# ydixon/yolo_v3

Hardware: AMD Instinct MI355X
Metric: images/sec (YOLOv3 forward + decode + NMS, 416x416, bs=64 per GPU) (higher is better)
Workload: dtype f32 (exact fp32 MFMA); 1 GPU; 416x416 bs=64 per GPU, 64 distinct synthetic scenes per GPU, SW-1 synthetic weights, conf=0.50 nms=0.40; global_batch=64, parallelism=dp1, entry=Detector.run_device, lanes=2

## Files before the change

### include/yv3.h

```cpp
#ifndef YV3_H
#define YV3_H

#include <stddef.h>
#include <stdint.h>

#ifdef __cplusplus
extern "C" {
#endif

#define YV3_VERSION 100

#define YV3_EINVAL   (-1)
#define YV3_ESHAPE   (-2)
#define YV3_EWORKSPACE (-3)
#define YV3_EDTYPE   (-4)
#define YV3_ERCCL    (-5)
#define YV3_ELIMIT   (-6)

#define YV3_F32  0
#define YV3_BF16 1
#define YV3_F32_BF16X3 2
#define YV3_F32_F16X2 3

#define YV3_ACT_LINEAR 0
#define YV3_ACT_LEAKY  1

int yv3_version(void);
const char* yv3_error_string(int code);


int yv3_pack_conv_weight(const float* w_oihw, void* w_packed, int cout, int cin, int k,
                         int cout_pad, int dtype, void* stream);

int yv3_fold_bn(const float* gamma, const float* bias, const float* mean, const float* var,
                float eps, float* alpha, float* beta, int channels, void* stream);

int yv3_split_planes(const float* in, void* out, long long n, int np, void* stream);
int yv3_merge_planes(const void* in, float* out, long long n, int np, void* stream);


int yv3_conv0(const float* x_nchw, const float* w_tap_major, const float* alpha, const float* beta,
              void* y_nhwc, int B, int H, int W, int out_dtype, int* flags, void* stream);

int yv3_conv_front(const float* x_nchw, const float* w0_tap_major, const float* alpha0, const float* beta0,
                   const void* w1_packed, const float* alpha1, const float* beta1, void* y,
                   int B, int H, int W, int* flags, void* stream);
int yv3_conv_front_bf16(const float* x_nchw, const float* w0_tap_major, const float* alpha0, const float* beta0,
                        const void* w1_packed, const float* alpha1, const float* beta1, void* y,
                        int B, int H, int W, int* flags, void* stream);
int yv3_conv_front_f32(const float* x_nchw, const float* w0_tap_major, const float* alpha0, const float* beta0,
                       const float* w1_packed, const float* alpha1, const float* beta1, float* y,
                       int B, int H, int W, void* stream);

int yv3_res_block64(const void* x, const void* w1_packed, const float* alpha1, const float* beta1,
                    const void* w2_packed, const float* alpha2, const float* beta2, void* y,
                    int B, int H, int W, int* flags, void* stream);
int yv3_res_block64_bf16(const void* x, const void* w1_packed, const float* alpha1, const float* beta1,
                         const void* w2_packed, const float* alpha2, const float* beta2, void* y,
                         int B, int H, int W, int* flags, void* stream);
int yv3_res_block64_f32(const float* x, const float* w1_packed, const float* alpha1, const float* beta1,
                        const float* w2_packed, const float* alpha2, const float* beta2, float* y,
                        int B, int H, int W, void* stream);

typedef struct yv3_conv_desc {
    const void*  x;
    const void*  x2;
    const void*  w;
    const float* alpha;
    const float* beta;
    const void*  residual;
    void*        y;
    int B, H, W;
    int cin;
    int cin_up;
    int cout, cout_pad;
    int k, stride;
    int act;
    int dtype;
    int out_dtype;
    int* flags;
    void*  workspace;
    size_t workspace_bytes;
    float*    dec_out;
    long long dec_out_batch_stride;
    float     dec_stride;
    float     dec_anchors[6];
    unsigned  options;
    int       big_tile_min;
    int       tune[4];
    long long x_plane_stride, x2_plane_stride, y_plane_stride;
    const void*  w_wino;
    const float* alpha_wino;
    void*        wino_ws;
    size_t       wino_ws_bytes;
    const void*  w_wino4;
} yv3_conv_desc;

#define YV3_OPT_NO_PINGPONG 1u
#define YV3_OPT_K3S1        2u
#define YV3_OPT_WINO_EVEN   4u
#define YV3_OPT_WINO_ALWAYS 8u
#define YV3_OPT_TWO_LANES   16u
#define YV3_OPT_WINO4_TILES 32u
#define YV3_OPT_TILE_SHIFT  8

size_t yv3_conv_workspace_bytes(void);

size_t yv3_wino_workspace_bytes(int B, int H, int W, int cin);

size_t yv3_wino4_workspace_bytes(int B, int H, int W, int cin);
int yv3_pack_wino4_weight_f32(const float* u_oc66, float* packed, int cout, int cin, void* stream);

int yv3_conv2d(const yv3_conv_desc* desc, void* stream);

#define YV3_FORM_DIRECT   0
#define YV3_FORM_WINOGRAD 1
#define YV3_FORM_WINOGRAD4 2
int yv3_conv2d_form(const yv3_conv_desc* desc);

int yv3_conv2d_launches(const yv3_conv_desc* desc);

int yv3_conv2d_kernel(const yv3_conv_desc* desc, char* buf, size_t buf_bytes);

int yv3_conv2d_sequence(const yv3_conv_desc* descs, int n, void* stream);


int yv3_decode(const float* logits, int ld_logits, const float* anchors_host, float stride,
               float* out, long long out_batch_stride, int B, int H, int W, int num_class,
               void* stream);

int yv3_decode_nchw(const float* logits_nchw, const float* anchors_host, float stride,
                    float* out, long long out_batch_stride, int B, int H, int W, int num_class,
                    void* stream);


int yv3_cxcywh_to_xyxy(const float* in, float* out, long long n, void* stream);

int yv3_iou_matrix(const float* b1, int n1, int ld1, const float* b2, int n2, int ld2,
                   int mode, float* out, void* stream);


size_t yv3_postproc_cand_bytes(int B, int max_cand, int num_class);

size_t yv3_postproc_nms_workspace_bytes(int B, int max_n, int num_class);

#define YV3_PP_EVAL 1
#define YV3_PP_PROB 2

int yv3_postproc_filter(const float* dets, int B, int N, int num_class, float conf_thr,
                        int mode, void* cand, int max_cand, int* cand_counts, void* stream);

int yv3_postproc_nms(const float* dets, int B, int N, int num_class, float nms_thr, int use_nms,
                     const void* cand, int max_cand, const int* cand_counts, int max_n,
                     float* out_boxes, int cap, int* out_counts,
                     void* workspace, size_t workspace_bytes, void* stream);


int yv3_letterbox(const unsigned char* img_hwc, int H, int W, float* out_chw, int out_h, int out_w,
                  void* stream);

int yv3_letterbox_ex(const unsigned char* img_hwc, int H, int W, float* out_chw, int out_h, int out_w,
                     int box_w, int box_h, int box_x, int box_y, void* stream);

int yv3_resize_linear(const unsigned char* img_hwc, int H, int W, float* out_chw, int out_h, int out_w,
                      void* stream);

int yv3_correct_boxes(const float* boxes, int B, int cap, int ld, const int* counts, const int* org_wh,
                      int img_w, int img_h, int is_letterbox, int out_xyxy, float* out, void* stream);


size_t yv3_augment_workspace_bytes(long long src_bytes);

int yv3_augment_images(const unsigned char* src, long long src_bytes, const long long* offsets, const int* hw,
                       const double* params, int B, float* out, int out_h, int out_w,
                       void* workspace, size_t workspace_bytes, int* status, void* stream);

int yv3_augment_labels(const double* labels, int B, int T, const int* hw, const double* params,
                       float* target, int max_rows, int out_h, int out_w, int* status, void* stream);

int yv3_upsample2x_concat(const float* up, const float* tail, float* out, int B, int c_up, int c_tail, int h, int w, void* stream);

int yv3_gather_boxes(const float* payload, float* gathered, int b_local, int rows, void* rccl_comm, void* stream);

#define YV3_COCO_MAX_MAXDETS 8

typedef struct yv3_cocoeval_desc {
    int n_gt, n_det, n_img, n_cat;
    const int* gt_img;
    const int* gt_cat;
    const double* gt_box;
    const double* gt_area;
    const int* gt_crowd;
    const long long* gt_id;
    const int* det_img;
    const int* det_cat;
    const double* det_box;
    const double* det_score;
    int n_iou, n_rec, n_area, n_maxdet;
    const double* iou_thrs;
    const double* rec_thrs;
    const double* area_rng;
    int max_dets[YV3_COCO_MAX_MAXDETS];
    double* precision;
    double* recall;
    double* scores;
    int* status;
} yv3_cocoeval_desc;

size_t yv3_cocoeval_workspace_bytes(int n_gt, int n_det, int n_img, int n_cat, int n_area);

int yv3_cocoeval(const yv3_cocoeval_desc* desc, void* ws, size_t ws_bytes, void* stream);

#define YV3_YOLO_LOSS_MAX_ROWS 1024

typedef struct yv3_yolo_loss_desc {
    const float* logits;
    float* grad;
    long long stride_b, stride_p, stride_c;
    const float* target;
    int B, H, W, T, num_class;
    float img_dim_h;
    float anchors[18];
    int mask[3];
    double* sums;
    int* counts;
    int* status;
} yv3_yolo_loss_desc;

size_t yv3_yolo_loss_workspace_bytes(int B, int H, int W, int T);

int yv3_yolo_loss(const yv3_yolo_loss_desc* desc, void* ws, size_t ws_bytes, void* stream);


int yv3_train_pack_weight(const float* w, float* wf, float* wd, int cout, int cin, int k, void* stream);

int yv3_train_conv_fwd(const float* x, const float* x2, const float* wf, const float* bias, float* z,
                       int B, int H, int W, int cin, int cin_up, int cout, int k, int stride, int x_nchw, void* stream);

int yv3_train_conv_dgrad(const float* dz, const float* wd, float* dx, int B, int H, int W, int cin, int cout, int k, int stride,
                         int accumulate, void* stream);

size_t yv3_train_conv_wgrad_workspace_bytes(int B, int H, int W, int cin, int cout, int k, int stride);
int yv3_train_conv_wgrad(const float* x, const float* x2, const float* dz, float* dw, int B, int H, int W, int cin, int cin_up,
                         int cout, int k, int stride, int x_nchw, void* ws, size_t ws_bytes, void* stream);

size_t yv3_train_channel_workspace_bytes(long long P, int C);

int yv3_train_bn_stats(const float* z, long long P, int C, float eps, float momentum, const float* run_mean, const float* run_var,
                       float* run_mean_out, float* run_var_out, float* mean, float* invstd, void* ws, size_t ws_bytes, void* stream);

int yv3_train_bn_eval_stats(const float* run_mean, const float* run_var, float eps, float* mean, float* invstd, int C, void* stream);

int yv3_train_bn_act_fwd(const float* z, const float* mean, const float* invstd, const float* gamma, const float* beta,
                         const float* residual, float* y, long long P, int C, void* stream);

int yv3_train_bn_act_bwd(const float* z, const float* dy, const float* mean, const float* invstd, const float* gamma, const float* beta,
// ... 30 lines not shown
```

### yolo_v3_amd/_ffi.py

```python
import ctypes
import os

_HERE = os.path.dirname(os.path.abspath(__file__))
LIB_PATH = (os.environ.get("YV3_LIB") if os.environ.get("YV3_MEASURE") == "1" else None) or os.path.join(_HERE, "libyv3.so")

if os.environ.get("YV3_MEASURE") != "1":
    _stray = sorted(k for k in os.environ if k.startswith("YV3_") and k not in ("YV3_MEASURE", "YV3_DIST_BACKEND", "YV3_DUMP_PLAN"))
    if _stray:
        import warnings
        warnings.warn("yolo_v3_amd: %s set but ignored -- library / kernel-selection overrides are honoured in measurement sessions only "
                      "(YV3_MEASURE=1); the bundled libyv3.so and the default plans are used" % ", ".join(_stray), RuntimeWarning)

F32, BF16, F32X3, F32H2 = 0, 1, 2, 3
ACT_LINEAR, ACT_LEAKY = 0, 1
PP_EVAL, PP_PROB = 1, 2
OPT_NO_PINGPONG, OPT_K3S1, OPT_WINO_EVEN, OPT_WINO_ALWAYS, OPT_TWO_LANES, OPT_WINO4_TILES = 1, 2, 4, 8, 16, 32
OPT_TILE_SHIFT = 8
(TILE_AUTO, TILE_256x128_W8, TILE_128x128_W8, TILE_128x128_W4, TILE_128x64, TILE_256x128_W4, TILE_256x256, TILE_256x128_W4_ROLL,
 TILE_256x256_ROLL, TILE_256x256_ROLL4) = range(10)
TILE_192x256_ROLL, TILE_W4_192x128, TILE_256x256_PP3, TILE_256x256_PP4, TILE_192x256_PP3, TILE_192x256_PP4 = 11, 12, 13, 14, 15, 16
T0_F32_TILE_64, T0_F32_TILE_128_W4, T0_F32_TILE_128_1X1, T0_WINO2_HALF, T0_WINO2_FULL = 2, 6, 7, 8, 9
T0_WINO4_NEVER, T0_WINO4_ALWAYS, T0_GEMM_NEVER, T0_GEMM_ALWAYS = 10, 11, 13, 14
T1_WINO4_NO_EVEN, T1_WINO4_NO_FULL, T1_GEMM_ALL_ROWS = 1, 2, 3
T1P_NO_SHORT_K, T1P_WINO_OTHER_LOOP, T1P_BF16_ROUND3, T1P_BF16_NO_192, T1P_NO_W4 = 1, 2, 8, 16, 32
T1P_NO_W4_1X1, T1P_NO_W4_3X3, T1P_W4_LANES_3X3, T1P_BF16_ROLL, T1P_BF16_PP3 = 64, 128, 256, 512, 1024
KERNEL_LINE_BYTES = 96


def conv2d_kernel(desc):
    buf = ctypes.create_string_buffer(KERNEL_LINE_BYTES)
    check(lib().yv3_conv2d_kernel(ctypes.byref(desc), buf, KERNEL_LINE_BYTES), "yv3_conv2d_kernel")
    return buf.value.decode()

c_void_p, c_int, c_float, c_size_t, c_longlong = (ctypes.c_void_p, ctypes.c_int, ctypes.c_float,
                                                  ctypes.c_size_t, ctypes.c_longlong)


class ConvDesc(ctypes.Structure):
    _fields_ = [("x", c_void_p), ("x2", c_void_p), ("w", c_void_p), ("alpha", c_void_p), ("beta", c_void_p),
                ("residual", c_void_p), ("y", c_void_p),
                ("B", c_int), ("H", c_int), ("W", c_int), ("cin", c_int), ("cin_up", c_int),
                ("cout", c_int), ("cout_pad", c_int), ("k", c_int), ("stride", c_int), ("act", c_int),
                ("dtype", c_int), ("out_dtype", c_int), ("flags", c_void_p),
                ("workspace", c_void_p), ("workspace_bytes", ctypes.c_size_t),
                ("dec_out", c_void_p), ("dec_out_batch_stride", c_longlong), ("dec_stride", c_float),
                ("dec_anchors", c_float * 6), ("options", ctypes.c_uint), ("big_tile_min", c_int), ("tune", c_int * 4),
                ("x_plane_stride", c_longlong), ("x2_plane_stride", c_longlong), ("y_plane_stride", c_longlong),
                ("w_wino", c_void_p), ("alpha_wino", c_void_p), ("wino_ws", c_void_p), ("wino_ws_bytes", ctypes.c_size_t),
                ("w_wino4", c_void_p)]


COCO_MAX_MAXDETS = 8
ELIMIT = -6


class CocoEvalDesc(ctypes.Structure):
    _fields_ = [("n_gt", c_int), ("n_det", c_int), ("n_img", c_int), ("n_cat", c_int),
                ("gt_img", c_void_p), ("gt_cat", c_void_p), ("gt_box", c_void_p), ("gt_area", c_void_p),
                ("gt_crowd", c_void_p), ("gt_id", c_void_p),
                ("det_img", c_void_p), ("det_cat", c_void_p), ("det_box", c_void_p), ("det_score", c_void_p),
                ("n_iou", c_int), ("n_rec", c_int), ("n_area", c_int), ("n_maxdet", c_int),
                ("iou_thrs", c_void_p), ("rec_thrs", c_void_p), ("area_rng", c_void_p),
                ("max_dets", c_int * COCO_MAX_MAXDETS),
                ("precision", c_void_p), ("recall", c_void_p), ("scores", c_void_p), ("status", c_void_p)]


YOLO_LOSS_MAX_ROWS = 1024
EINVAL, ESHAPE, EWORKSPACE = -1, -2, -3


class YoloLossDesc(ctypes.Structure):
    _fields_ = [("logits", c_void_p), ("grad", c_void_p),
                ("stride_b", c_longlong), ("stride_p", c_longlong), ("stride_c", c_longlong),
                ("target", c_void_p), ("B", c_int), ("H", c_int), ("W", c_int), ("T", c_int), ("num_class", c_int),
                ("img_dim_h", c_float), ("anchors", c_float * 18), ("mask", c_int * 3),
                ("sums", c_void_p), ("counts", c_void_p), ("status", c_void_p)]


_SIGNATURES = {
    "yv3_version": (c_int, []),
    "yv3_conv_workspace_bytes": (ctypes.c_size_t, []),
    "yv3_wino_workspace_bytes": (ctypes.c_size_t, [c_int, c_int, c_int, c_int]),
    "yv3_wino4_workspace_bytes": (ctypes.c_size_t, [c_int, c_int, c_int, c_int]),
    "yv3_pack_wino4_weight_f32": (c_int, [c_void_p, c_void_p, c_int, c_int, c_void_p]),
    "yv3_error_string": (ctypes.c_char_p, [c_int]),
    "yv3_pack_conv_weight": (c_int, [c_void_p, c_void_p, c_int, c_int, c_int, c_int, c_int, c_void_p]),
    "yv3_fold_bn": (c_int, [c_void_p, c_void_p, c_void_p, c_void_p, c_float, c_void_p, c_void_p, c_int, c_void_p]),
    "yv3_split_planes": (c_int, [c_void_p, c_void_p, c_longlong, c_int, c_void_p]),
    "yv3_merge_planes": (c_int, [c_void_p, c_void_p, c_longlong, c_int, c_void_p]),
    "yv3_conv0": (c_int, [c_void_p, c_void_p, c_void_p, c_void_p, c_void_p, c_int, c_int, c_int, c_int, c_void_p, c_void_p]),
    "yv3_conv_front": (c_int, [c_void_p, c_void_p, c_void_p, c_void_p, c_void_p, c_void_p, c_void_p, c_void_p, c_int, c_int, c_int, c_void_p, c_void_p]),
    "yv3_conv_front_bf16": (c_int, [c_void_p, c_void_p, c_void_p, c_void_p, c_void_p, c_void_p, c_void_p, c_void_p, c_int, c_int, c_int, c_void_p, c_void_p]),
    "yv3_res_block64": (c_int, [c_void_p, c_void_p, c_void_p, c_void_p, c_void_p, c_void_p, c_void_p, c_void_p, c_int, c_int, c_int, c_void_p, c_void_p]),
    "yv3_res_block64_bf16": (c_int, [c_void_p, c_void_p, c_void_p, c_void_p, c_void_p, c_void_p, c_void_p, c_void_p, c_int, c_int, c_int, c_void_p, c_void_p]),
    "yv3_conv_front_f32": (c_int, [c_void_p, c_void_p, c_void_p, c_void_p, c_void_p, c_void_p, c_void_p, c_void_p, c_int, c_int, c_int, c_void_p]),
    "yv3_res_block64_f32": (c_int, [c_void_p, c_void_p, c_void_p, c_void_p, c_void_p, c_void_p, c_void_p, c_void_p, c_int, c_int, c_int, c_void_p]),
    "yv3_conv2d": (c_int, [ctypes.POINTER(ConvDesc), c_void_p]),
    "yv3_conv2d_form": (c_int, [ctypes.POINTER(ConvDesc)]),
    "yv3_conv2d_launches": (c_int, [ctypes.POINTER(ConvDesc)]),
    "yv3_conv2d_kernel": (c_int, [ctypes.POINTER(ConvDesc), ctypes.c_char_p, c_size_t]),
    "yv3_conv2d_sequence": (c_int, [ctypes.POINTER(ConvDesc), c_int, c_void_p]),
    "yv3_decode": (c_int, [c_void_p, c_int, ctypes.POINTER(c_float), c_float, c_void_p, c_longlong,
                           c_int, c_int, c_int, c_int, c_void_p]),
    "yv3_decode_nchw": (c_int, [c_void_p, ctypes.POINTER(c_float), c_float, c_void_p, c_longlong,
                                c_int, c_int, c_int, c_int, c_void_p]),
    "yv3_cxcywh_to_xyxy": (c_int, [c_void_p, c_void_p, c_longlong, c_void_p]),
    "yv3_iou_matrix": (c_int, [c_void_p, c_int, c_int, c_void_p, c_int, c_int, c_int, c_void_p, c_void_p]),
    "yv3_letterbox": (c_int, [c_void_p, c_int, c_int, c_void_p, c_int, c_int, c_void_p]),
    "yv3_letterbox_ex": (c_int, [c_void_p, c_int, c_int, c_void_p, c_int, c_int, c_int, c_int, c_int, c_int, c_void_p]),
    "yv3_resize_linear": (c_int, [c_void_p, c_int, c_int, c_void_p, c_int, c_int, c_void_p]),
    "yv3_augment_workspace_bytes": (c_size_t, [c_longlong]),
    "yv3_augment_images": (c_int, [c_void_p, c_longlong, c_void_p, c_void_p, c_void_p, c_int, c_void_p, c_int, c_int,
                                   c_void_p, c_size_t, c_void_p, c_void_p]),
    "yv3_augment_labels": (c_int, [c_void_p, c_int, c_int, c_void_p, c_void_p, c_void_p, c_int, c_int, c_int, c_void_p, c_void_p]),
    "yv3_upsample2x_concat": (c_int, [c_void_p, c_void_p, c_void_p, c_int, c_int, c_int, c_int, c_int, c_void_p]),
    "yv3_correct_boxes": (c_int, [c_void_p, c_int, c_int, c_int, c_void_p, c_void_p, c_int, c_int, c_int, c_int, c_void_p, c_void_p]),
    "yv3_gather_boxes": (c_int, [c_void_p, c_void_p, c_int, c_int, c_void_p, c_void_p]),
    "yv3_postproc_cand_bytes": (c_size_t, [c_int, c_int, c_int]),
    "yv3_postproc_nms_workspace_bytes": (c_size_t, [c_int, c_int, c_int]),
    "yv3_postproc_filter": (c_int, [c_void_p, c_int, c_int, c_int, c_float, c_int, c_void_p, c_int, c_void_p, c_void_p]),
    "yv3_postproc_nms": (c_int, [c_void_p, c_int, c_int, c_int, c_float, c_int, c_void_p, c_int, c_void_p, c_int,
                                 c_void_p, c_int, c_void_p, c_void_p, c_size_t, c_void_p]),
    "yv3_cocoeval_workspace_bytes": (c_size_t, [c_int, c_int, c_int, c_int, c_int]),
    "yv3_cocoeval": (c_int, [ctypes.POINTER(CocoEvalDesc), c_void_p, c_size_t, c_void_p]),
    "yv3_yolo_loss_workspace_bytes": (c_size_t, [c_int, c_int, c_int, c_int]),
    "yv3_yolo_loss": (c_int, [ctypes.POINTER(YoloLossDesc), c_void_p, c_size_t, c_void_p]),
    "yv3_train_pack_weight": (c_int, [c_void_p, c_void_p, c_void_p, c_int, c_int, c_int, c_void_p]),
    "yv3_train_conv_fwd": (c_int, [c_void_p, c_void_p, c_void_p, c_void_p, c_void_p] + [c_int] * 9 + [c_void_p]),
    "yv3_train_conv_dgrad": (c_int, [c_void_p, c_void_p, c_void_p] + [c_int] * 8 + [c_void_p]),
    "yv3_train_conv_wgrad_workspace_bytes": (c_size_t, [c_int] * 7),
    "yv3_train_conv_wgrad": (c_int, [c_void_p, c_void_p, c_void_p, c_void_p] + [c_int] * 9 + [c_void_p, c_size_t, c_void_p]),
    "yv3_train_channel_workspace_bytes": (c_size_t, [c_longlong, c_int]),
    "yv3_train_bn_stats": (c_int, [c_void_p, c_longlong, c_int, c_float, c_float] + [c_void_p] * 7 + [c_size_t, c_void_p]),
    "yv3_train_bn_eval_stats": (c_int, [c_void_p, c_void_p, c_float, c_void_p, c_void_p, c_int, c_void_p]),
    "yv3_train_bn_act_fwd": (c_int, [c_void_p] * 7 + [c_longlong, c_int, c_void_p]),
    "yv3_train_bn_act_bwd": (c_int, [c_void_p] * 9 + [c_longlong, c_int, c_int, c_void_p, c_size_t, c_void_p]),
    "yv3_train_bias_bwd": (c_int, [c_void_p] * 4 + [c_longlong, c_int, c_void_p, c_size_t, c_void_p]),
    "yv3_train_add": (c_int, [c_void_p, c_void_p, c_longlong, c_void_p]),
    "yv3_train_upcat_bwd": (c_int, [c_void_p] * 3 + [c_int] * 7 + [c_void_p]),
    "yv3_train_to_bf16": (c_int, [c_void_p, c_void_p, c_longlong, c_int, c_int, c_void_p]),
    "yv3_train_pack_weight_bf16": (c_int, [c_void_p, c_void_p, c_void_p, c_int, c_int, c_int, c_void_p]),
    "yv3_train_conv_fwd_bf16": (c_int, [c_void_p, c_void_p, c_void_p, c_void_p, c_void_p] + [c_int] * 9 + [c_void_p]),
    "yv3_train_conv_dgrad_bf16": (c_int, [c_void_p, c_void_p, c_void_p] + [c_int] * 8 + [c_void_p]),
    "yv3_train_conv_wgrad_bf16_workspace_bytes": (c_size_t, [c_int] * 7),
    "yv3_train_conv_wgrad_bf16": (c_int, [c_void_p, c_void_p, c_void_p, c_void_p] + [c_int] * 9 + [c_void_p, c_size_t, c_void_p]),
}

EXPORTS = tuple(_SIGNATURES)
_lib = None


class Yv3Error(RuntimeError):
    code = None


class GpuOnlyError(Yv3Error, NotImplementedError):
    """A CPU tensor where only the GPU path exists (the reference's training branch runs on CPU tensors; this package does not)."""


def lib():
    global _lib
    if _lib is None:
        if not os.path.exists(LIB_PATH):
            raise Yv3Error("HIP extension %s is missing: build it with "
                           "`python -c 'import __graft_entry__ as g; g.build()'` "
                           "(or `make -C yolo_v3_amd/csrc`). There is no CPU fallback." % LIB_PATH)
        handle = ctypes.CDLL(LIB_PATH)
        for name, (res, args) in _SIGNATURES.items():
            fn = getattr(handle, name)
# ... 25 lines not shown
```

### yolo_v3_amd/csrc/conv_wino4_f32.hip

```cpp
#include <type_traits>
#include "yv3_common.h"

namespace {

#define W4F_GPTR(p) ((const __attribute__((address_space(1))) void*)(p))
#define W4F_LPTR(p) ((__attribute__((address_space(3))) void*)(p))

typedef float f32x2 __attribute__((ext_vector_type(2)));

constexpr int BNC = 64;
constexpr int BMT = 32;
constexpr int ROWB = 128;
constexpr int U_BYTES = BNC * ROWB;
constexpr int V_BYTES = BMT * ROWB;
constexpr int STAGE = U_BYTES + V_BYTES;
#define W4F_NSTAGE 4
#ifndef W4F_PRIO
#define W4F_PRIO 3
#endif
#ifndef W4F_EXTRA_LDS
#define W4F_EXTRA_LDS 0
#endif
#ifndef W4F_DMA_FIRST
#define W4F_DMA_FIRST 0
#endif
constexpr int NSTAGE = W4F_NSTAGE;
#if defined(YV3_MEASURE) && defined(W4F_ABL)
constexpr int ABL = W4F_ABL;
#else
constexpr int ABL = 0;
#endif

struct Wino4Params {
    const float* v;
    const float* u;
    const float* alpha;
    const float* beta;
    const float* res;
    float* y;
    int C, Cout, H, W, th, tw, T;
    int cchunks;
    int nblk_n;
    int act;
    long long pos_stride;
    unsigned u_bytes, v_bytes;
    int nitems, n_full, parts;
    float* sk_parts;
    int* sk_flags;
    int* status;
};
constexpr int W4F_MAX_TAIL_WG = 2 * YV3_WINO_SK_MAX_WG - 1;
constexpr int W4F_PART_FLOATS = 4 * 32 * 256;

template <int N> __device__ __forceinline__ void w4f_wait_vmcnt() { asm volatile("s_waitcnt vmcnt(%0)" :: "n"(N) : "memory"); }

__device__ __forceinline__ int w4f_swz(int row) { return (row >> 1) & 7; }

__device__ __forceinline__ void bt_apply(const f32x4 (&d)[6], f32x4 (&o)[6]) {
    o[0] = d[0] - 1.5f * d[1] - 2.0f * d[2] + 1.5f * d[3] + d[4];
    o[1] = 0.5f * d[2] - d[1] + 2.5f * d[3] + d[4];
    o[2] = d[1] - 2.5f * d[2] + 0.5f * d[3] + d[4];
    o[3] = 2.0f * (d[3] - d[1]) - d[2] + d[4];
    o[4] = 0.5f * (d[1] - d[3]) - d[2] + d[4];
    o[5] = d[1] - 1.5f * d[2] - 2.0f * d[3] + 1.5f * d[4] + d[5];
}

__global__ __launch_bounds__(256) void wino4_input_f32_kernel(const float* __restrict__ x, float* __restrict__ v,
                                                              int H, int W, int C, int th, int tw, long long T) {
    const int cg = C >> 2;
    const long long i = (long long)blockIdx.x * blockDim.x + threadIdx.x;
    if (i >= T * cg) return;
    const long long t = i / cg;
    const int c = (int)(i - t * cg) * 4;
    const int b = (int)(t / (th * tw));
    const int rem = (int)(t - (long long)b * th * tw);
    const int ty = rem / tw, tx = rem - ty * tw;
    const int y0 = 4 * ty - 1, x0 = 4 * tx - 1;
    f32x4 tr[6][6];
#pragma unroll
    for (int r = 0; r < 6; ++r) {
        f32x4 d[6];
        const int yy = y0 + r;
#pragma unroll
        for (int q = 0; q < 6; ++q) {
            const int xx = x0 + q;
            const bool ok = (unsigned)yy < (unsigned)H && (unsigned)xx < (unsigned)W;
            d[q] = ok ? *reinterpret_cast<const f32x4*>(x + (((long long)b * H + yy) * W + xx) * C + c) : f32x4{0.f, 0.f, 0.f, 0.f};
        }
        bt_apply(d, tr[r]);
    }
#pragma unroll
    for (int l = 0; l < 6; ++l) {
        f32x4 col[6], o[6];
#pragma unroll
        for (int r = 0; r < 6; ++r) col[r] = tr[r][l];
        bt_apply(col, o);
#pragma unroll
        for (int xi = 0; xi < 6; ++xi) *reinterpret_cast<f32x4*>(v + ((long long)(xi * 6 + l) * T + t) * C + c) = o[xi];
    }
}

__global__ __launch_bounds__(256) void wino4_pack_kernel(const float* __restrict__ u, float* __restrict__ out, int cout, int cin) {
    const long long i = (long long)blockIdx.x * blockDim.x + threadIdx.x;
    const long long n4 = (long long)cout * cin * 36 / 4;
    if (i >= n4) return;
    const int cch = cin / 32;
    const int ps = (int)(i & 7);
    const int row = (int)((i >> 3) & 63);
    long long r = i >> 9;
    const int cc = (int)(r % cch); r /= cch;
    const int pos = (int)(r % 36);
    const int nb = (int)(r / 36);
    const int slot = ps ^ w4f_swz(row);
    const int o = nb * 64 + row, c = cc * 32 + slot * 4;
    f32x4 q;
#pragma unroll
    for (int e = 0; e < 4; ++e) q[e] = u[((long long)o * cin + c + e) * 36 + pos];
    *reinterpret_cast<f32x4*>(out + i * 4) = q;
}

__device__ __forceinline__ constexpr float at_coef(int j, int nu) {
    return nu == 0 ? (j == 0 ? 1.f : 0.f)
         : nu == 1 ? 1.f
         : nu == 2 ? ((j & 1) ? -1.f : 1.f)
         : nu == 3 ? (j == 0 ? 1.f : j == 1 ? 0.5f : j == 2 ? 0.25f : 0.125f)
         : nu == 4 ? (j == 0 ? 1.f : j == 1 ? -2.f : j == 2 ? 4.f : -8.f)
         : (j == 3 ? 1.f : 0.f);
}

template <bool CCH2, bool SK>
__global__ __launch_bounds__(256, 2) void conv_wino4_f32_kernel(const Wino4Params p) {
    extern __shared__ __attribute__((aligned(16))) unsigned char lds[];
    const int tid = threadIdx.x;
    const int lane = tid & 63;
    const int wid = __builtin_amdgcn_readfirstlane(tid >> 6);
    const int nk = 36 * p.cchunks;
    const int nkx = 6 * p.cchunks;
#if defined(YV3_MEASURE) && defined(W4F_DEPHASE)
    if (blockIdx.x >= 256 && blockIdx.x < 512)
        for (int i = 0; i < nk * W4F_DEPHASE / 5000; ++i) __builtin_amdgcn_s_sleep(108);
#endif

    int item, xa = 0, xb = 6, sk_t = 0;
    if (!SK || (int)blockIdx.x < p.n_full) item = yv3_xcd_remap(blockIdx.x, SK ? p.n_full : (int)gridDim.x);
    else {
        sk_t = blockIdx.x - p.n_full;
        const int nt = p.nitems - p.n_full;
        const int x = sk_t & 7, l = sk_t >> 3;
        const int i0 = (int)(((long long)nt * x) >> 3), i1 = (int)(((long long)nt * (x + 1)) >> 3);
        const int il = l / p.parts, part = l - il * p.parts;
        if (il >= i1 - i0) return;
        item = p.n_full + i0 + il;
        const int rows = 6 / p.parts;
        xa = part * rows; xb = xa + rows;
    }

    const __amdgpu_buffer_rsrc_t urs = __builtin_amdgcn_make_buffer_rsrc(const_cast<float*>(p.u), 0, (int)p.u_bytes, 0x00020000);
    const __amdgpu_buffer_rsrc_t vrs = __builtin_amdgcn_make_buffer_rsrc(const_cast<float*>(p.v), 0, (int)p.v_bytes, 0x00020000);
    unsigned usoff = 0;
    const unsigned uoff = lane * 16;
    unsigned vsoff = 0, voff = 0;
    int pf_c = 0;
    int pf_k = 0, pf_end = 0;
    auto dma_piece = [&](int i, unsigned char* stage) {
        if (ABL & 8) return;
        if (i == 0)      __builtin_amdgcn_raw_ptr_buffer_load_lds(urs, W4F_LPTR(stage + (2 * wid) * 1024), 16, uoff, usoff, 0, 0);
        else if (i == 1) __builtin_amdgcn_raw_ptr_buffer_load_lds(urs, W4F_LPTR(stage + (2 * wid) * 1024), 16, uoff, usoff, 1024, 0);
        else             __builtin_amdgcn_raw_ptr_buffer_load_lds(vrs, W4F_LPTR(stage + U_BYTES + wid * 1024), 16, voff, vsoff, 0, 0);
    };
    auto dma_advance = [&]() {
        if (pf_k + 1 < pf_end) {
            ++pf_k;
            usoff += BNC * 32 * 4;
            vsoff += 128;
            pf_c += 32;
            if (pf_c == p.C) { pf_c = 0; vsoff += (unsigned)(p.pos_stride - p.C) * 4u; }
        }
    };

    const int fr = lane & 15, fq = lane >> 4;
    const int urow = 16 * wid + fr;
    const int u_off0 = urow * ROWB + ((fq ^ w4f_swz(urow)) << 4);
    const int u_off1 = urow * ROWB + (((4 + fq) ^ w4f_swz(urow)) << 4);
    int v_off0[2], v_off1[2];
#pragma unroll
    for (int b = 0; b < 2; ++b) {
        const int r = 16 * b + fr;
        v_off0[b] = U_BYTES + r * ROWB + ((fq ^ w4f_swz(r)) << 4);
        v_off1[b] = U_BYTES + r * ROWB + (((4 + fq) ^ w4f_swz(r)) << 4);
    }

    f32x4 P[2], R[4][2], Y[4][4][2];
    struct Frag { f32x4 ua, va0, va1, ub, vb0, vb1; };
    auto read_frag = [&](const unsigned char* st) {
        Frag f;
        if (ABL & 4) { f.ua = f.va0 = f.va1 = f.ub = f.vb0 = f.vb1 = f32x4{(float)lane, 1.f, 2.f, 3.f}; return f; }
        f.ua = *reinterpret_cast<const f32x4*>(st + u_off0);
        f.va0 = *reinterpret_cast<const f32x4*>(st + v_off0[0]);
        f.va1 = *reinterpret_cast<const f32x4*>(st + v_off0[1]);
        f.ub = *reinterpret_cast<const f32x4*>(st + u_off1);
        f.vb0 = *reinterpret_cast<const f32x4*>(st + v_off1[0]);
        f.vb1 = *reinterpret_cast<const f32x4*>(st + v_off1[1]);
        return f;
    };
    Frag F0, F1;
    using TrueT = std::integral_constant<bool, true>;
    using FalseT = std::integral_constant<bool, false>;

#if defined(YV3_MEASURE) && defined(W4F_TIMELINE)
    unsigned long long tl_t = __builtin_amdgcn_s_memtime(), tl_sync = 0, tl_burst = 0, tl_fold = 0;
    const unsigned long long tl_entry = tl_t;
#define W4F_MARK(acc_) do { const unsigned long long t_ = __builtin_amdgcn_s_memtime(); acc_ += t_ - tl_t; tl_t = t_; } while (0)
#else
#define W4F_MARK(acc_) do {} while (0)
#endif
    auto chunk = [&](auto first_c, auto stage_c, const Frag& F, Frag& G) {
        constexpr bool FIRST = decltype(first_c)::value;
        constexpr int S = decltype(stage_c)::value;
        const f32x4 zero4 = {0.f, 0.f, 0.f, 0.f};
        W4F_MARK(tl_fold);
        w4f_wait_vmcnt<3 * (NSTAGE - 2)>();
        __builtin_amdgcn_s_waitcnt(0xC07F);
        if (!(ABL & 16)) __builtin_amdgcn_s_barrier();
        __builtin_amdgcn_sched_barrier(0);
        W4F_MARK(tl_sync);
        unsigned char* const fr_ = lds + S * STAGE;
        G = read_frag(lds + ((S + 1) % NSTAGE) * STAGE);
#if W4F_PRIO == 3
        __builtin_amdgcn_s_setprio(1);
#endif
#pragma unroll
        for (int t = 0; t < 4; ++t) {
            if (ABL & 2) { P[0][t] += F.ua[t] + F.va0[t]; P[1][t] += F.va1[t]; }
            else {
            P[0] = __builtin_amdgcn_mfma_f32_16x16x4f32(F.ua[t], F.va0[t], (FIRST && t == 0) ? zero4 : P[0], 0, 0, 0);
            P[1] = __builtin_amdgcn_mfma_f32_16x16x4f32(F.ua[t], F.va1[t], (FIRST && t == 0) ? zero4 : P[1], 0, 0, 0);
            }
            __builtin_amdgcn_sched_barrier(0);
            if (t < 3) dma_piece(t, fr_);
            __builtin_amdgcn_sched_barrier(0);
        }
#pragma unroll
        for (int t = 0; t < 4; ++t) {
            if (ABL & 2) { P[0][t] += F.ub[t] + F.vb0[t]; P[1][t] += F.vb1[t]; }
            else {
            P[0] = __builtin_amdgcn_mfma_f32_16x16x4f32(F.ub[t], F.vb0[t], P[0], 0, 0, 0);
            P[1] = __builtin_amdgcn_mfma_f32_16x16x4f32(F.ub[t], F.vb1[t], P[1], 0, 0, 0);
            }
        }
#if W4F_PRIO == 3
        __builtin_amdgcn_s_setprio(0);
#endif
        dma_advance();
        W4F_MARK(tl_burst);
    };

    auto position = [&](auto nu_c) {
        constexpr int nu = decltype(nu_c)::value;
        {
            using S0 = std::integral_constant<int, 0>; using S1 = std::integral_constant<int, 1>;
            using S2 = std::integral_constant<int, 2>; using S3 = std::integral_constant<int, 3>;
            if constexpr (CCH2) {
                if constexpr ((nu & 1) == 0) { chunk(TrueT{}, S0{}, F0, F1); chunk(FalseT{}, S1{}, F1, F0); }
                else                         { chunk(TrueT{}, S2{}, F0, F1); chunk(FalseT{}, S3{}, F1, F0); }
            } else {
                chunk(TrueT{}, S0{}, F0, F1); chunk(FalseT{}, S1{}, F1, F0); chunk(FalseT{}, S2{}, F0, F1); chunk(FalseT{}, S3{}, F1, F0);
                for (int cc = 4; cc < p.cchunks; cc += 4) {
                    chunk(FalseT{}, S0{}, F0, F1); chunk(FalseT{}, S1{}, F1, F0); chunk(FalseT{}, S2{}, F0, F1); chunk(FalseT{}, S3{}, F1, F0);
                }
            }
            if (ABL & 32) return;
#pragma unroll
            for (int b = 0; b < 2; ++b) {
#pragma unroll
                for (int j = 0; j < 4; ++j) {
                    constexpr float z = 0.f;
                    const float cf = at_coef(j, nu);
                    if (cf != z) {
#pragma unroll
                        for (int e = 0; e < 4; ++e) R[j][b][e] = fmaf(P[b][e], cf, R[j][b][e]);
                    }
                }
            }
        }
    };
    {
        const int nb = item % p.nblk_n;
        const int n0 = nb * BNC;
        const int m0 = (item / p.nblk_n) * BMT;
        {
            const int k0 = xa * nkx;
            usoff = (unsigned)((((long long)nb * nk + k0) * (BNC * 32) + (2 * wid) * 256) * 4);
            const int vrow = 8 * wid + (lane >> 3);
            const int vt = min(m0 + vrow, p.T - 1);
            vsoff = (unsigned)m0 * (unsigned)p.C * 4u + (unsigned)(6 * xa) * (unsigned)p.pos_stride * 4u;
            voff = (unsigned)(vt - m0) * (unsigned)p.C * 4u + ((((unsigned)lane & 7u) ^ (unsigned)w4f_swz(vrow)) << 4);
            pf_c = 0; pf_k = k0; pf_end = xb * nkx;
        }
#pragma unroll
        for (int b = 0; b < 2; ++b) {
            P[b] = f32x4{0.f, 0.f, 0.f, 0.f};
#pragma unroll
            for (int j = 0; j < 4; ++j) {
                R[j][b] = f32x4{0.f, 0.f, 0.f, 0.f};
#pragma unroll
                for (int i = 0; i < 4; ++i) Y[i][j][b] = f32x4{0.f, 0.f, 0.f, 0.f};
            }
        }
#pragma unroll
        for (int d = 0; d < NSTAGE; ++d) {
#pragma unroll
            for (int i = 0; i < 3; ++i) dma_piece(i, lds + d * STAGE);
            dma_advance();
        }
        w4f_wait_vmcnt<3 * (NSTAGE - 1)>();
        __builtin_amdgcn_s_barrier();
#if W4F_PRIO == 1
        if (__builtin_amdgcn_s_getreg((3 << 11) | 4) & 1) __builtin_amdgcn_s_setprio(2);
#elif W4F_PRIO == 2
        if ((blockIdx.x >> 8) & 1) __builtin_amdgcn_s_setprio(2);
#endif
        F0 = read_frag(lds);
        for (int xi = xa; xi < xb; ++xi) {
            position(std::integral_constant<int, 0>{}); position(std::integral_constant<int, 1>{}); position(std::integral_constant<int, 2>{});
            position(std::integral_constant<int, 3>{}); position(std::integral_constant<int, 4>{}); position(std::integral_constant<int, 5>{});
            const float c1 = xi == 0 || xi == 5 ? 0.f : xi == 1 ? 1.f : xi == 2 ? -1.f : xi == 3 ? 0.5f : -2.f;
            const float cfi[4] = {xi == 5 ? 0.f : 1.f, c1, c1 * c1, xi == 5 ? 1.f : c1 * c1 * c1};
#pragma unroll
            for (int i = 0; i < 4; ++i) {
                if (cfi[i] == 0.f) continue;
#pragma unroll
                for (int j = 0; j < 4; ++j)
#pragma unroll
                    for (int b = 0; b < 2; ++b)
#pragma unroll
                        for (int e = 0; e < 4; ++e) Y[i][j][b][e] = fmaf(R[j][b][e], cfi[i], Y[i][j][b][e]);
            }
#pragma unroll
            for (int j = 0; j < 4; ++j)
#pragma unroll
                for (int b = 0; b < 2; ++b) R[j][b] = f32x4{0.f, 0.f, 0.f, 0.f};
        }
        w4f_wait_vmcnt<0>();
#if defined(YV3_MEASURE) && defined(W4F_TIMELINE)
        const unsigned long long tl_loop_end = __builtin_amdgcn_s_memtime();
#endif

        if constexpr (SK) {
            if (xa == 0 && xb < 6) {
                for (int k = 1; k < p.parts; ++k) {
                    const int partner = sk_t + 8 * k;
                    if (tid == 0) {
                        int n = 0, f;
                        while ((f = __hip_atomic_load(p.sk_flags + partner, __ATOMIC_RELAXED, __HIP_MEMORY_SCOPE_AGENT)) == 0 && ++n < (1 << 22))
                            __builtin_amdgcn_s_sleep(2);
                        if ((f == 0 || f != 1 + (int)(__builtin_amdgcn_s_getreg((3 << 11) | 20) & 15)) && p.status) atomicOr(p.status, 2);
                        __hip_atomic_store(p.sk_flags + partner, 0, __ATOMIC_RELAXED, __HIP_MEMORY_SCOPE_AGENT);
                    }
                    __syncthreads();
                    const float* w = p.sk_parts + (size_t)partner * W4F_PART_FLOATS + wid * (32 * 256) + lane * 4;
#pragma unroll
                    for (int i = 0; i < 4; ++i) {
                        f32x4 t[4][2];
#pragma unroll
                        for (int j = 0; j < 4; ++j)
#pragma unroll
                            for (int b = 0; b < 2; ++b) t[j][b] = *reinterpret_cast<const f32x4*>(w + ((i * 4 + j) * 2 + b) * 256);
#pragma unroll
                        for (int j = 0; j < 4; ++j)
#pragma unroll
                            for (int b = 0; b < 2; ++b) Y[i][j][b] += t[j][b];
                        __builtin_amdgcn_sched_barrier(0);
                    }
                }
            }
        }

        const bool raw = SK && xa > 0;
        const int cw = n0 + 16 * wid + 4 * fq;
        const f32x4 one4 = {1.f, 1.f, 1.f, 1.f}, zero4 = {0.f, 0.f, 0.f, 0.f};
        const f32x4 al = raw ? one4 : *reinterpret_cast<const f32x4*>(p.alpha + cw);
        const f32x4 be = raw ? zero4 : *reinterpret_cast<const f32x4*>(p.beta + cw);
        const bool leaky = !raw && p.act == YV3_ACT_LEAKY;
        const float* const res = raw ? nullptr : p.res;
        float* const ybase = raw ? p.sk_parts + (size_t)sk_t * W4F_PART_FLOATS + wid * (32 * 256) + lane * 4 : p.y;
        long long pix[2];
        int py[2], px[2];
#pragma unroll
        for (int b = 0; b < 2; ++b) {
            const int t = m0 + 16 * b + fr;
            if (t < p.T) {
                const int tt = p.th * p.tw;
                const int bi = t / tt, rem = t - bi * tt;
                const int ty = rem / p.tw, tx = rem - ty * p.tw;
                py[b] = 4 * ty; px[b] = 4 * tx;
                pix[b] = ((long long)bi * p.H + py[b]) * p.W + px[b];
            } else { pix[b] = -1; py[b] = px[b] = 0; }
        }
        auto out_off = [&](int i, int j, int b) -> long long {
            if (raw) return ((i * 4 + j) * 2 + b) * 256;
            const bool ok = pix[b] >= 0 && py[b] + i < p.H && px[b] + j < p.W;
            return ok ? (pix[b] + (long long)i * p.W + j) * p.Cout + cw : -1;
        };
        f32x4 rr[2][4][2];
        auto load_res = [&](int i) {
#pragma unroll
            for (int j = 0; j < 4; ++j)
#pragma unroll
                for (int b = 0; b < 2; ++b) {
                    const long long off = out_off(i, j, b);
                    rr[i & 1][j][b] = off >= 0 ? *reinterpret_cast<const f32x4*>(res + off) : f32x4{0.f, 0.f, 0.f, 0.f};
                }
        };
        if (res) load_res(0);
#pragma unroll
        for (int i = 0; i < ((ABL & 1) ? 1 : 4); ++i) {
            if (res && i + 1 < 4) load_res(i + 1);
#pragma unroll
            for (int j = 0; j < 4; ++j)
#pragma unroll
                for (int b = 0; b < 2; ++b) {
                    const long long off = out_off(i, j, b);
                    f32x4 q;
#pragma unroll
                    for (int e = 0; e < 4; ++e) {
                        float v = fmaf(Y[i][j][b][e], al[e], be[e]);
                        if (leaky) v = v > 0.f ? v : 0.1f * v;
                        q[e] = res ? v + rr[i & 1][j][b][e] : v;
                    }
                    if (off >= 0) *reinterpret_cast<f32x4*>(ybase + off) = q;
                }
        }
        if (raw) {
            asm volatile("s_waitcnt vmcnt(0)" ::: "memory");
            __syncthreads();
            if (tid == 0) __hip_atomic_store(p.sk_flags + sk_t, 1 + (int)(__builtin_amdgcn_s_getreg((3 << 11) | 20) & 15),
                                             __ATOMIC_RELAXED, __HIP_MEMORY_SCOPE_AGENT);
        }
#if defined(YV3_MEASURE) && defined(W4F_TIMELINE)
        if (blockIdx.x == W4F_TIMELINE && lane == 0) {
            const unsigned long long tl_end = __builtin_amdgcn_s_memtime();
            __builtin_amdgcn_s_waitcnt(0);
            float* dbg = p.y + wid * 8;
            dbg[0] = (float)tl_sync / nk; dbg[1] = (float)tl_burst / nk; dbg[2] = (float)tl_fold / nk; dbg[3] = (float)(tl_loop_end - tl_entry);
            dbg[4] = (float)(tl_end - tl_loop_end); dbg[5] = (float)nk;
        }
#endif
    }
}

}

extern "C" int yv3_pack_wino4_weight_f32(const float* u_oc66, float* packed, int cout, int cin, void* stream) {
    if (!u_oc66 || !packed || cout <= 0 || cin <= 0) return YV3_EINVAL;
    if (cout % 64 || (cin != 64 && cin % 128)) return YV3_ESHAPE;
    const long long n4 = (long long)cout * cin * 9;
    hipLaunchKernelGGL(wino4_pack_kernel, dim3((unsigned)((n4 + 255) / 256)), dim3(256), 0, (hipStream_t)stream, u_oc66, packed, cout, cin);
    YV3_CHECK_LAUNCH();
    return 0;
}

static_assert(BMT == YV3_SEL_WINO4_TILES && BNC == YV3_SEL_WINO4_CHANNELS && W4F_MAX_TAIL_WG == YV3_SEL_WINO4_MAX_TAIL_WG && ROWB == 4 * YV3_SEL_CHUNK,
              "conv_select.cpp counts this kernel's items, tail workgroups and chunks");

extern "C" size_t yv3_wino4_workspace_bytes(int B, int H, int W, int cin) {
    if (B <= 0 || H <= 0 || W <= 0 || cin <= 0) return 0;
    return yv3_wino4_ws_bytes(B, H, W, cin);
}

int yv3_conv2d_wino4_f32(const yv3_conv_desc* d, const yv3_f32_choice& c, hipStream_t s) {
    const int th = (d->H + 3) / 4, tw = (d->W + 3) / 4;
    const long long T = (long long)d->B * th * tw;
    float* v = (float*)d->wino_ws;
    {
        const long long n = T * (d->cin >> 2);
        hipLaunchKernelGGL(wino4_input_f32_kernel, dim3((unsigned)((n + 255) / 256)), dim3(256), 0, s, (const float*)d->x, v, d->H, d->W, d->cin, th, tw, T);
        YV3_CHECK_LAUNCH();
    }
    Wino4Params p;
    p.v = v; p.u = (const float*)d->w_wino4;
    p.alpha = d->alpha; p.beta = d->beta; p.res = (const float*)d->residual; p.y = (float*)d->y;
    p.C = d->cin; p.Cout = d->cout; p.H = d->H; p.W = d->W; p.th = th; p.tw = tw; p.T = (int)T;
    p.cchunks = d->cin / 32; p.nblk_n = c.ntiles; p.act = d->act;
    p.pos_stride = T * d->cin;
    p.u_bytes = (unsigned)(36ull * d->cout * d->cin * 4); p.v_bytes = (unsigned)(36ull * T * d->cin * 4);
    const long long items = ((T + BMT - 1) / BMT) * p.nblk_n;
    p.nitems = (int)items;
    p.n_full = c.n_full; p.parts = c.parts;
    char* area = (char*)d->wino_ws + ((d->wino_ws_bytes - yv3_wino_sk_bytes()) & ~(size_t)255);
    p.sk_parts = (float*)area;
    p.sk_flags = (int*)(area + (size_t)W4F_MAX_TAIL_WG * W4F_PART_FLOATS * sizeof(float));
    p.status = d->flags;
    const size_t lds = (size_t)NSTAGE * STAGE + W4F_EXTRA_LDS;
    if (p.parts > 1) {
        const long long tail = items - p.n_full;
        const dim3 grid((unsigned)(p.n_full + 8 * ((tail + 7) / 8) * p.parts));
        if (p.cchunks == 2) hipLaunchKernelGGL((conv_wino4_f32_kernel<true, true>), grid, dim3(256), lds, s, p);
        else                hipLaunchKernelGGL((conv_wino4_f32_kernel<false, true>), grid, dim3(256), lds, s, p);
    } else {
        const dim3 grid((unsigned)items);
        if (p.cchunks == 2) hipLaunchKernelGGL((conv_wino4_f32_kernel<true, false>), grid, dim3(256), lds, s, p);
        else                hipLaunchKernelGGL((conv_wino4_f32_kernel<false, false>), grid, dim3(256), lds, s, p);
    }
    YV3_CHECK_LAUNCH();
    return 0;
}
```

Before: 3297 images/sec.

## Store Winograd F(4,3) output rows 0-2 early, overlapping with the last transform position

In the non-split-K Winograd-4 fp32 kernel, the epilogue for output rows 0-2 now runs before the final input-transform position (xi=5). Only row 3 receives that position's contribution, so those stores and residual loads overlap with the last position's MMA chunks. The epilogue becomes a macro that takes a row range. Chunk waits at the start of the next position are skipped for stages already covered by the drained pipeline. An option bit restores the late store, and the split-K path keeps the old schedule. This adds register pressure and more complex scheduling, and stores issued mid-pipeline may compete with the loads.

```diff
diff --git a/include/yv3.h b/include/yv3.h
--- a/include/yv3.h
+++ b/include/yv3.h
@@ -102,6 +102,7 @@
 #define YV3_OPT_WINO_ALWAYS 8u
 #define YV3_OPT_TWO_LANES   16u
 #define YV3_OPT_WINO4_TILES 32u
+#define YV3_OPT_WINO4_LATE_STORE 64u
 #define YV3_OPT_TILE_SHIFT  8
 
 size_t yv3_conv_workspace_bytes(void);
diff --git a/yolo_v3_amd/_ffi.py b/yolo_v3_amd/_ffi.py
--- a/yolo_v3_amd/_ffi.py
+++ b/yolo_v3_amd/_ffi.py
@@ -15,6 +15,7 @@
 ACT_LINEAR, ACT_LEAKY = 0, 1
 PP_EVAL, PP_PROB = 1, 2
 OPT_NO_PINGPONG, OPT_K3S1, OPT_WINO_EVEN, OPT_WINO_ALWAYS, OPT_TWO_LANES, OPT_WINO4_TILES = 1, 2, 4, 8, 16, 32
+OPT_WINO4_LATE_STORE = 64
 OPT_TILE_SHIFT = 8
 (TILE_AUTO, TILE_256x128_W8, TILE_128x128_W8, TILE_128x128_W4, TILE_128x64, TILE_256x128_W4, TILE_256x256, TILE_256x128_W4_ROLL,
  TILE_256x256_ROLL, TILE_256x256_ROLL4) = range(10)
diff --git a/yolo_v3_amd/csrc/conv_wino4_f32.hip b/yolo_v3_amd/csrc/conv_wino4_f32.hip
--- a/yolo_v3_amd/csrc/conv_wino4_f32.hip
+++ b/yolo_v3_amd/csrc/conv_wino4_f32.hip
@@ -23,6 +23,9 @@
 #endif
 #ifndef W4F_DMA_FIRST
 #define W4F_DMA_FIRST 0
+#endif
+#ifndef W4F_EARLY_ROWS
+#define W4F_EARLY_ROWS 1
 #endif
 constexpr int NSTAGE = W4F_NSTAGE;
 #if defined(YV3_MEASURE) && defined(W4F_ABL)
@@ -128,8 +131,71 @@
          : (j == 3 ? 1.f : 0.f);
 }
 
-template <bool CCH2, bool SK>
+#define W4F_EPILOGUE(LO_, HI_) do { \
+        constexpr int LO = (LO_), HI = (HI_); \
+        constexpr bool ROWWAIT = (EARLY && W4F_EARLY_ROWS != 3) || (!SK && W4F_EARLY_ROWS == 4); \
+        const bool raw = SK && xa > 0; \
+        const int cw = n0 + 16 * wid + 4 * fq; \
+        const f32x4 one4 = {1.f, 1.f, 1.f, 1.f}, zero4 = {0.f, 0.f, 0.f, 0.f}; \
+        const f32x4 al = raw ? one4 : *reinterpret_cast<const f32x4*>(p.alpha + cw); \
+        const f32x4 be = raw ? zero4 : *reinterpret_cast<const f32x4*>(p.beta + cw); \
+        const bool leaky = !raw && p.act == YV3_ACT_LEAKY; \
+        const float* const res = raw ? nullptr : p.res; \
+        float* const ybase = raw ? p.sk_parts + (size_t)sk_t * W4F_PART_FLOATS + wid * (32 * 256) + lane * 4 : p.y; \
+        long long pix[2]; \
+        int py[2], px[2]; \
+        _Pragma("unroll") \
+        for (int b = 0; b < 2; ++b) { \
+            const int t = m0 + 16 * b + fr; \
+            if (t < p.T) { \
+                const int tt = p.th * p.tw; \
+                const int bi = t / tt, rem = t - bi * tt; \
+                const int ty = rem / p.tw, tx = rem - ty * p.tw; \
+                py[b] = 4 * ty; px[b] = 4 * tx; \
+                pix[b] = ((long long)bi * p.H + py[b]) * p.W + px[b]; \
+            } else { pix[b] = -1; py[b] = px[b] = 0; } \
+        } \
+        auto out_off = [&](int i, int j, int b) -> long long { \
+            if (raw) return ((i * 4 + j) * 2 + b) * 256; \
+            const bool ok = pix[b] >= 0 && py[b] + i < p.H && px[b] + j < p.W; \
+            return ok ? (pix[b] + (long long)i * p.W + j) * p.Cout + cw : -1; \
+        }; \
+        f32x4 rr[2][4][2]; \
+        auto load_res = [&](int i) { \
+        _Pragma("unroll") \
+            for (int j = 0; j < 4; ++j) \
+        _Pragma("unroll") \
+                for (int b = 0; b < 2; ++b) { \
+                    const long long off = out_off(i, j, b); \
+                    rr[i & 1][j][b] = off >= 0 ? *reinterpret_cast<const f32x4*>(res + off) : f32x4{0.f, 0.f, 0.f, 0.f}; \
+                } \
+        }; \
+        constexpr int END = (ABL & 1) ? (LO == 0 ? 1 : LO) : HI; \
+        if (res && LO < END) load_res(LO); \
+        _Pragma("unroll") \
+        for (int i = LO; i < END; ++i) { \
+            if (res && i + 1 < END) load_res(i + 1); \
+            if (ROWWAIT && (i == LO || i + 1 < END)) __builtin_amdgcn_s_waitcnt(0x0F70); \
+        _Pragma("unroll") \
+            for (int j = 0; j < 4; ++j) \
+        _Pragma("unroll") \
+                for (int b = 0; b < 2; ++b) { \
+                    const long long off = out_off(i, j, b); \
+                    f32x4 q; \
+        _Pragma("unroll") \
+                    for (int e = 0; e < 4; ++e) { \
+                        float v = fmaf(Y[i][j][b][e], al[e], be[e]); \
+                        if (leaky) v = v > 0.f ? v : 0.1f * v; \
+                        q[e] = res ? v + rr[i & 1][j][b][e] : v; \
+                    } \
+                    if (off >= 0) *reinterpret_cast<f32x4*>(ybase + off) = q; \
+                } \
+        } \
+    } while (0)
+
+template <bool CCH2, bool SK, bool EARLY = false>
 __global__ __launch_bounds__(256, 2) void conv_wino4_f32_kernel(const Wino4Params p) {
+    static_assert(!(SK && EARLY), "a part's Y is not final before the hand-over: the even schedule keeps the late epilogue");
     extern __shared__ __attribute__((aligned(16))) unsigned char lds[];
     const int tid = threadIdx.x;
     const int lane = tid & 63;
@@ -208,18 +274,19 @@
     using FalseT = std::integral_constant<bool, false>;
 
 #if defined(YV3_MEASURE) && defined(W4F_TIMELINE)
-    unsigned long long tl_t = __builtin_amdgcn_s_memtime(), tl_sync = 0, tl_burst = 0, tl_fold = 0;
+    unsigned long long tl_t = __builtin_amdgcn_s_memtime(), tl_sync = 0, tl_burst = 0, tl_fold = 0, tl_early = 0, tl_row5 = 0;
     const unsigned long long tl_entry = tl_t;
 #define W4F_MARK(acc_) do { const unsigned long long t_ = __builtin_amdgcn_s_memtime(); acc_ += t_ - tl_t; tl_t = t_; } while (0)
 #else
 #define W4F_MARK(acc_) do {} while (0)
 #endif
-    auto chunk = [&](auto first_c, auto stage_c, const Frag& F, Frag& G) {
+    auto chunk = [&](auto first_c, auto stage_c, const Frag& F, Frag& G, auto wait_c) {
         constexpr bool FIRST = decltype(first_c)::value;
         constexpr int S = decltype(stage_c)::value;
+        constexpr bool WAIT = decltype(wait_c)::value;
         const f32x4 zero4 = {0.f, 0.f, 0.f, 0.f};
         W4F_MARK(tl_fold);
-        w4f_wait_vmcnt<3 * (NSTAGE - 2)>();
+        if constexpr (WAIT) w4f_wait_vmcnt<3 * (NSTAGE - 2)>();
         __builtin_amdgcn_s_waitcnt(0xC07F);
         if (!(ABL & 16)) __builtin_amdgcn_s_barrier();
         __builtin_amdgcn_sched_barrier(0);
@@ -255,18 +322,22 @@
         W4F_MARK(tl_burst);
     };
 
-    auto position = [&](auto nu_c) {
+#define W4F_W(c_) std::integral_constant<bool, ((c_) >= SKIP)>{}
+    auto position = [&](auto nu_c, auto skip_c) {
         constexpr int nu = decltype(nu_c)::value;
+        constexpr int SKIP = decltype(skip_c)::value;
         {
             using S0 = std::integral_constant<int, 0>; using S1 = std::integral_constant<int, 1>;
             using S2 = std::integral_constant<int, 2>; using S3 = std::integral_constant<int, 3>;
             if constexpr (CCH2) {
-                if constexpr ((nu & 1) == 0) { chunk(TrueT{}, S0{}, F0, F1); chunk(FalseT{}, S1{}, F1, F0); }
-                else                         { chunk(TrueT{}, S2{}, F0, F1); chunk(FalseT{}, S3{}, F1, F0); }
+                if constexpr ((nu & 1) == 0) { chunk(TrueT{}, S0{}, F0, F1, W4F_W(0)); chunk(FalseT{}, S1{}, F1, F0, W4F_W(1)); }
+                else                         { chunk(TrueT{}, S2{}, F0, F1, W4F_W(0)); chunk(FalseT{}, S3{}, F1, F0, W4F_W(1)); }
             } else {
-                chunk(TrueT{}, S0{}, F0, F1); chunk(FalseT{}, S1{}, F1, F0); chunk(FalseT{}, S2{}, F0, F1); chunk(FalseT{}, S3{}, F1, F0);
+                chunk(TrueT{}, S0{}, F0, F1, W4F_W(0)); chunk(FalseT{}, S1{}, F1, F0, W4F_W(1)); chunk(FalseT{}, S2{}, F0, F1, W4F_W(2));
+                chunk(FalseT{}, S3{}, F1, F0, W4F_W(3));
                 for (int cc = 4; cc < p.cchunks; cc += 4) {
-                    chunk(FalseT{}, S0{}, F0, F1); chunk(FalseT{}, S1{}, F1, F0); chunk(FalseT{}, S2{}, F0, F1); chunk(FalseT{}, S3{}, F1, F0);
+                    chunk(FalseT{}, S0{}, F0, F1, TrueT{}); chunk(FalseT{}, S1{}, F1, F0, TrueT{}); chunk(FalseT{}, S2{}, F0, F1, TrueT{});
+                    chunk(FalseT{}, S3{}, F1, F0, TrueT{});
                 }
             }
             if (ABL & 32) return;
@@ -321,9 +392,10 @@
         if ((blockIdx.x >> 8) & 1) __builtin_amdgcn_s_setprio(2);
 #endif
         F0 = read_frag(lds);
-        for (int xi = xa; xi < xb; ++xi) {
-            position(std::integral_constant<int, 0>{}); position(std::integral_constant<int, 1>{}); position(std::integral_constant<int, 2>{});
-            position(std::integral_constant<int, 3>{}); position(std::integral_constant<int, 4>{}); position(std::integral_constant<int, 5>{});
+        using I0 = std::integral_constant<int, 0>; using I1 = std::integral_constant<int, 1>; using I2 = std::integral_constant<int, 2>;
+        using I3 = std::integral_constant<int, 3>; using I4 = std::integral_constant<int, 4>; using I5 = std::integral_constant<int, 5>;
+        for (int xi = xa; xi < (EARLY ? 5 : xb); ++xi) {
+            position(I0{}, I0{}); position(I1{}, I0{}); position(I2{}, I0{}); position(I3{}, I0{}); position(I4{}, I0{}); position(I5{}, I0{});
             const float c1 = xi == 0 || xi == 5 ? 0.f : xi == 1 ? 1.f : xi == 2 ? -1.f : xi == 3 ? 0.5f : -2.f;
             const float cfi[4] = {xi == 5 ? 0.f : 1.f, c1, c1 * c1, xi == 5 ? 1.f : c1 * c1 * c1};
 #pragma unroll
@@ -340,6 +412,44 @@
             for (int j = 0; j < 4; ++j)
 #pragma unroll
                 for (int b = 0; b < 2; ++b) R[j][b] = f32x4{0.f, 0.f, 0.f, 0.f};
+        }
+        if constexpr (EARLY) {
+            auto early_rows = [&](auto lo_c, auto hi_c) {
+                constexpr int LO_ = decltype(lo_c)::value, HI_ = decltype(hi_c)::value;
+                W4F_MARK(tl_fold);
+                w4f_wait_vmcnt<0>();
+                W4F_EPILOGUE(LO_, LO_ + 1);
+                if constexpr (LO_ + 1 < HI_) W4F_EPILOGUE(LO_ + 1, HI_);
+                __builtin_amdgcn_sched_barrier(0);
+                W4F_MARK(tl_early);
+            };
+            constexpr int SK0 = CCH2 ? 2 : NSTAGE - 1, SK1 = CCH2 ? NSTAGE - 3 : 0;
+            using K0 = std::integral_constant<int, SK0>; using K1 = std::integral_constant<int, SK1>;
+            static_assert(NSTAGE == 4, "SK0 + SK1 == NSTAGE - 1 chunks run without a wait");
+#if defined(YV3_MEASURE) && defined(W4F_TIMELINE)
+            const unsigned long long tl_row5_0 = __builtin_amdgcn_s_memtime(), tl_early_0 = tl_early;
+#endif
+#if W4F_EARLY_ROWS == 2
+            position(I0{}, I0{});
+            early_rows(I0{}, I1{});
+            position(I1{}, K0{}); position(I2{}, K1{});
+            early_rows(I1{}, I2{});
+            position(I3{}, K0{}); position(I4{}, K1{});
+            early_rows(I2{}, I3{});
+            position(I5{}, K0{});
+#else
+            early_rows(I0{}, I3{});
+            position(I0{}, K0{}); position(I1{}, K1{}); position(I2{}, I0{}); position(I3{}, I0{}); position(I4{}, I0{}); position(I5{}, I0{});
+#endif
+#if defined(YV3_MEASURE) && defined(W4F_TIMELINE)
+            tl_row5 = __builtin_amdgcn_s_memtime() - tl_row5_0 - (tl_early - tl_early_0);
+#endif
+#pragma unroll
+            for (int j = 0; j < 4; ++j)
+#pragma unroll
+                for (int b = 0; b < 2; ++b)
+#pragma unroll
+                    for (int e = 0; e < 4; ++e) Y[3][j][b][e] = fmaf(R[j][b][e], 1.f, Y[3][j][b][e]);
         }
         w4f_wait_vmcnt<0>();
 #if defined(YV3_MEASURE) && defined(W4F_TIMELINE)
@@ -376,62 +486,8 @@
             }
         }
 
-        const bool raw = SK && xa > 0;
-        const int cw = n0 + 16 * wid + 4 * fq;
-        const f32x4 one4 = {1.f, 1.f, 1.f, 1.f}, zero4 = {0.f, 0.f, 0.f, 0.f};
-        const f32x4 al = raw ? one4 : *reinterpret_cast<const f32x4*>(p.alpha + cw);
-        const f32x4 be = raw ? zero4 : *reinterpret_cast<const f32x4*>(p.beta + cw);
-        const bool leaky = !raw && p.act == YV3_ACT_LEAKY;
-        const float* const res = raw ? nullptr : p.res;
-        float* const ybase = raw ? p.sk_parts + (size_t)sk_t * W4F_PART_FLOATS + wid * (32 * 256) + lane * 4 : p.y;
-        long long pix[2];
-        int py[2], px[2];
-#pragma unroll
-        for (int b = 0; b < 2; ++b) {
-            const int t = m0 + 16 * b + fr;
-            if (t < p.T) {
-                const int tt = p.th * p.tw;
-                const int bi = t / tt, rem = t - bi * tt;
-                const int ty = rem / p.tw, tx = rem - ty * p.tw;
-                py[b] = 4 * ty; px[b] = 4 * tx;
-                pix[b] = ((long long)bi * p.H + py[b]) * p.W + px[b];
-            } else { pix[b] = -1; py[b] = px[b] = 0; }
-        }
-        auto out_off = [&](int i, int j, int b) -> long long {
-            if (raw) return ((i * 4 + j) * 2 + b) * 256;
-            const bool ok = pix[b] >= 0 && py[b] + i < p.H && px[b] + j < p.W;
-            return ok ? (pix[b] + (long long)i * p.W + j) * p.Cout + cw : -1;
-        };
-        f32x4 rr[2][4][2];
-        auto load_res = [&](int i) {
-#pragma unroll
-            for (int j = 0; j < 4; ++j)
-#pragma unroll
-                for (int b = 0; b < 2; ++b) {
-                    const long long off = out_off(i, j, b);
-                    rr[i & 1][j][b] = off >= 0 ? *reinterpret_cast<const f32x4*>(res + off) : f32x4{0.f, 0.f, 0.f, 0.f};
-                }
-        };
-        if (res) load_res(0);
-#pragma unroll
-        for (int i = 0; i < ((ABL & 1) ? 1 : 4); ++i) {
-            if (res && i + 1 < 4) load_res(i + 1);
-#pragma unroll
-            for (int j = 0; j < 4; ++j)
-#pragma unroll
-                for (int b = 0; b < 2; ++b) {
-                    const long long off = out_off(i, j, b);
-                    f32x4 q;
-#pragma unroll
-                    for (int e = 0; e < 4; ++e) {
-                        float v = fmaf(Y[i][j][b][e], al[e], be[e]);
-                        if (leaky) v = v > 0.f ? v : 0.1f * v;
-                        q[e] = res ? v + rr[i & 1][j][b][e] : v;
-                    }
-                    if (off >= 0) *reinterpret_cast<f32x4*>(ybase + off) = q;
-                }
-        }
-        if (raw) {
+        W4F_EPILOGUE(EARLY ? 3 : 0, 4);
+        if (SK && xa > 0) {
             asm volatile("s_waitcnt vmcnt(0)" ::: "memory");
             __syncthreads();
             if (tid == 0) __hip_atomic_store(p.sk_flags + sk_t, 1 + (int)(__builtin_amdgcn_s_getreg((3 << 11) | 20) & 15),
@@ -444,6 +500,7 @@
             float* dbg = p.y + wid * 8;
             dbg[0] = (float)tl_sync / nk; dbg[1] = (float)tl_burst / nk; dbg[2] = (float)tl_fold / nk; dbg[3] = (float)(tl_loop_end - tl_entry);
             dbg[4] = (float)(tl_end - tl_loop_end); dbg[5] = (float)nk;
+            dbg[6] = (float)tl_early; dbg[7] = (float)tl_row5;
         }
 #endif
     }
@@ -491,6 +548,8 @@
     p.sk_parts = (float*)area;
     p.sk_flags = (int*)(area + (size_t)W4F_MAX_TAIL_WG * W4F_PART_FLOATS * sizeof(float));
     p.status = d->flags;
+    const bool early = W4F_EARLY_ROWS >= 1 && W4F_EARLY_ROWS <= 3 && !(d->options & YV3_OPT_WINO4_LATE_STORE);
+    (void)early;
     const size_t lds = (size_t)NSTAGE * STAGE + W4F_EXTRA_LDS;
     if (p.parts > 1) {
         const long long tail = items - p.n_full;
@@ -499,6 +558,12 @@
         else                hipLaunchKernelGGL((conv_wino4_f32_kernel<false, true>), grid, dim3(256), lds, s, p);
     } else {
         const dim3 grid((unsigned)items);
+#if W4F_EARLY_ROWS
+        if (early) {
+            if (p.cchunks == 2) hipLaunchKernelGGL((conv_wino4_f32_kernel<true, false, true>), grid, dim3(256), lds, s, p);
+            else                hipLaunchKernelGGL((conv_wino4_f32_kernel<false, false, true>), grid, dim3(256), lds, s, p);
+        } else
+#endif
         if (p.cchunks == 2) hipLaunchKernelGGL((conv_wino4_f32_kernel<true, false>), grid, dim3(256), lds, s, p);
         else                hipLaunchKernelGGL((conv_wino4_f32_kernel<false, false>), grid, dim3(256), lds, s, p);
     }
```

Result: no change. 3307 images/sec (median of 6 runs) (+0.3%).
